# Liam-Eagen/BulletproofsPP

Measured on AMD Instinct MI355X. Metric: msm_scalar_point_pairs_per_sec, higher is better.
Workload: dtype u256 modular integer (Fq: 10x26-bit lazy limbs, Fr: 8x32-bit limbs); 1 GPU; pedersen_msm_2^20_secp256k1; pairs_per_gpu=1048576, window_bits=auto, algorithm=signed-digit Pippenger, affine in / XYZZ buckets

## Files before the change

### bulletproofspp_amd/capi.py

```python
from __future__ import annotations

import ctypes as C
import os
from typing import Optional, Sequence, Tuple

import numpy as np

_HERE = os.path.dirname(os.path.abspath(__file__))
NUM_STAGES = 6
STAGE_NAMES = ["digits", "sort", "acc_points", "acc_records", "reduce", "finish"]

SYMBOLS = [
    "bppp_ctx_create", "bppp_ctx_destroy", "bppp_ctx_set_stream", "bppp_last_error", "bppp_version",
    "bppp_msm", "bppp_msm_device", "bppp_msm_batch_device", "bppp_sum_points", "bppp_rational_reduce",
    "bppp_fold_points", "bppp_fold_points_device", "bppp_rational_reduce_eis", "bppp_fold_points_eis_device",
    "bppp_norm_round_sums_device", "bppp_lin_round_sums_device",
    "bppp_norm_round_openings_device", "bppp_lin_round_openings_device",
    "bppp_fold_scalars_device", "bppp_tensor_device", "bppp_batch_inverse_device",
    "bppp_nl_create", "bppp_nl_destroy", "bppp_nl_lengths", "bppp_nl_round_commit", "bppp_nl_round_collapse",
    "bppp_nl_get_witness", "bppp_nl_download", "bppp_nl_verify", "bppp_nl_verify_batch_device", "bppp_nl_prove", "bppp_nl_verify_challenges",
    "bppp_nlb_create", "bppp_nlb_destroy", "bppp_nlb_lengths", "bppp_nlb_round_commit", "bppp_nlb_round_collapse", "bppp_nlb_get_witness",
    "bppp_ip_create", "bppp_ip_destroy", "bppp_ip_lengths", "bppp_ip_round_commit", "bppp_ip_round_collapse", "bppp_ip_get_witness", "bppp_ip_verify", "bppp_ip_verify_batch_device",
    "bppp_lift_x_device", "bppp_device_alloc", "bppp_device_free", "bppp_upload", "bppp_download", "bppp_host_alloc", "bppp_host_free",
    "bppp_profile_enable", "bppp_profile_read",
# ... 229 lines not shown
    lib.bppp_rp_set_append.argtypes = [vp, sz, vp]
    lib.bppp_rp_set_info.argtypes = [vp, C.POINTER(C.c_uint64), C.POINTER(sz), C.POINTER(sz), C.POINTER(sz)]
    lib.bppp_rp_set_root.argtypes = [vp, vp]
    lib.bppp_rp_set_peaks.argtypes = [vp, vp]
    lib.bppp_rp_set_path_bytes.argtypes = [C.c_uint64]
    lib.bppp_rp_set_path_bytes.restype = sz
    lib.bppp_rp_set_paths.argtypes = [vp, sz, vp, vp]
    lib.bppp_rp_set_verify_paths.argtypes = [vp, sz, C.c_uint64, vp, sz, vp, vp, vp, vp, C.POINTER(C.c_int)]
    lib.bppp_seed_candidate_x.argtypes =[C.c_char_p, sz, C.c_uint64, vp]
    lib.bppp_points_from_seed.argtypes = [vp, C.c_char_p, sz, C.c_uint64, sz, vp, C.POINTER(C.c_uint64)]
    lib.bppp_points_from_seed_device.argtypes = [vp, C.c_char_p, sz, C.c_uint64, sz, vp, C.POINTER(C.c_uint64)]
    lib.bppp_rp_create_seeded.argtypes = [vp, i, i, vp, sz, vp, sz, C.c_char_p, sz, C.c_char_p, C.POINTER(vp)]
    lib.bppp_rp_create_binary_seeded.argtypes = [vp, i, i, vp, sz, vp, C.c_char_p, sz, C.c_char_p, C.POINTER(vp)]
    lib.bppp_profile_enable.argtypes = [vp, i]
    lib.bppp_profile_read.argtypes = [vp, C.POINTER(C.c_double), C.POINTER(C.c_uint64), i]
    return lib


def load_test_library() -> C.CDLL:
    p = os.path.join(_HERE, "lib", "libbppp_hip_test.so")
    if not os.path.exists(p):
        raise BpppError(f"{p} is missing: run `python -c 'import __graft_entry__ as g; g.build()'`")
    lib = C.CDLL(p)
    vp, sz, i = C.c_void_p, C.c_size_t, C.c_int
    lib.bppp_test_fe_op.argtypes = [vp, i, i, vp, vp, sz, vp]
    lib.bppp_test_point_op.argtypes = [vp, i, vp, vp, sz, vp]
    lib.bppp_test_point_quad.argtypes = [vp, i, vp, vp, sz, vp, vp]
    lib.bppp_test_fq_pair.argtypes = [vp, i, vp, vp, vp, vp, sz, vp]
    lib.bppp_test_point_chain.argtypes = [vp, i, vp, vp, sz, vp, vp]
    lib.bppp_test_mulmod_rate.argtypes = [vp, i, C.POINTER(C.c_double)]
    lib.bppp_test_last_mixed_msm_terms.argtypes = [vp, C.POINTER(C.c_uint64)]
    lib.bppp_test_last_sort_ranges.argtypes = [vp, C.POINTER(C.c_int)]
    lib.bppp_test_last_scatter_one_read.argtypes = [vp, C.POINTER(C.c_int)]
    lib.bppp_test_last_acc_sized.argtypes = [vp, C.POINTER(C.c_int)]
    lib.bppp_test_last_acc_fq29.argtypes = [vp, C.POINTER(C.c_int)]
    lib.bppp_test_fq29_op.argtypes = [vp, i, vp, vp, sz, vp, vp]
    lib.bppp_test_madd29_chain.argtypes = [vp, vp, vp, sz, sz, vp, vp]
    lib.bppp_test_madd26_chain.argtypes = [vp, vp, vp, sz, sz, vp, vp]
    lib.bppp_test_ec29_fast_op.argtypes = [vp, i, vp, sz, vp]
    lib.bppp_test_last_msm_layout.argtypes = [vp, C.POINTER(TestMsmLayout)]
    lib.bppp_test_last_msm_copy.argtypes = [vp, i, vp, sz]
    lib.bppp_test_last_windows.argtypes = [vp, C.POINTER(C.c_int)]
    lib.bppp_test_rp_last_verify_counts.argtypes = [vp, C.POINTER(C.c_uint64), C.POINTER(C.c_uint64)]
    lib.bppp_test_rp_last_block_counts.argtypes = [vp] + [C.POINTER(C.c_uint64)] * 4
    lib.bppp_test_rp_set_each_chunk.argtypes = [vp, sz]
    lib.bppp_test_rp_set_tally_short_max.argtypes = [vp, sz]
    lib.bppp_test_rp_set_tally_piece.argtypes = [vp, sz]
    lib.bppp_test_rp_set_tally_chunk.argtypes = [vp, sz]
    lib.bppp_test_rp_set_flat_chunk.argtypes = [vp, sz]
    lib.bppp_test_rp_excess_mul.argtypes = [vp, sz, vp, vp, vp]
    lib.bppp_test_rp_excess_mul2.argtypes = [vp, sz, vp, vp, vp, vp, vp]
    lib.bppp_test_rp_scan_mul.argtypes = [vp, sz, vp, vp, vp]
    lib.bppp_test_rp_scan_recode.argtypes = [vp, vp]
    lib.bppp_test_rp_scan_keys_mul.argtypes = [vp, sz, vp, sz, vp, vp]
    lib.bppp_test_rp_scan_keys_recode.argtypes = [vp, vp]
    lib.bppp_test_rp_scan_keys_geometry.argtypes = [vp, sz, sz, vp]
    lib.bppp_test_rp_witness_device.argtypes = [vp, sz, vp, vp, vp, vp, vp, vp, vp, vp, vp]
    lib.bppp_test_points_from_seed_chunked.argtypes = [vp, C.c_char_p, sz, C.c_uint64, sz, sz, vp, C.POINTER(C.c_uint64)]
    lib.bppp_test_seed_lift_digests.argtypes = [vp, C.c_char_p, sz, vp, vp, vp]
    lib.bppp_test_rp_decode_device.argtypes = [vp, sz, C.c_char_p, C.c_char_p, vp, vp, vp, vp, vp, vp]
    lib.bppp_test_comb_create.argtypes = [vp, vp, sz, i, C.POINTER(vp)]
    lib.bppp_test_comb_destroy.argtypes = [vp]
    lib.bppp_test_comb_destroy.restype = None
    lib.bppp_test_comb_msm.argtypes = [vp, vp, sz, sz, i, sz, vp]
    lib.bppp_test_comb_groups.argtypes = [vp, vp, sz, sz, sz, i, sz, vp]
    lib.bppp_test_comb_lanes.argtypes = [vp, vp, sz, sz, vp]
# ... 461 lines not shown
```

### bulletproofspp_amd/csrc/capi.hip

```cpp
#include <stdlib.h>
#include <string.h>
#include "ctx.hpp"
#include "hostmath.hpp"
#include "hosteis.hpp"

namespace bppp {
int msm_run(bppp_ctx *, const void *, const void *, size_t, size_t, int, int, uint64_t *);
int fold_points_run(bppp_ctx *, const uint64_t *, int, const uint64_t *, int, const void *, size_t, void *);
int norm_round_sums_run(bppp_ctx *, const void *, size_t, const uint64_t *, uint64_t *, uint64_t *);
int lin_round_sums_run(bppp_ctx *, const void *, const void *, size_t, uint64_t *, uint64_t *);
int round_openings_run(bppp_ctx *, const void *, size_t, int, const uint64_t *, const uint64_t *, void *, void *);
int fold_scalars_run(bppp_ctx *, const uint64_t *, const uint64_t *, const void *, size_t, void *);
int tensor_run(bppp_ctx *, const uint64_t *, size_t, const uint64_t *, const uint64_t *, size_t, void *);
int lift_x_run(bppp_ctx *, const void *, size_t, void *);
int batch_inverse_run(bppp_ctx *, const void *, size_t, int, void *);
int fold_points_eis_run(bppp_ctx *, const uint64_t *, const int *, const uint64_t *, const int *, const void *, size_t, void *);

void ctx_retain(bppp_ctx *ctx) { ctx->refs.fetch_add(1); }
void ctx_release(bppp_ctx *ctx) {
  if (ctx->refs.fetch_sub(1) != 1) return;
  hipSetDevice(ctx->device);
  hipStreamSynchronize(ctx->stream);
  if (ctx->aux_stream) hipStreamSynchronize(ctx->aux_stream);
  if (ctx->ws) hipFree(ctx->ws);
  if (ctx->ws2) hipFree(ctx->ws2);
  if (ctx->mix) hipFree(ctx->mix);
  if (ctx->pinned) hipHostFree(ctx->pinned);
  if (ctx->ev_ready) for (int i = 0; i <= BPPP_NUM_STAGES; i++) hipEventDestroy(ctx->ev[i]);
  if (ctx->aux_fork) hipEventDestroy(ctx->aux_fork);
  if (ctx->aux_join) hipEventDestroy(ctx->aux_join);
  if (ctx->aux_stream) hipStreamDestroy(ctx->aux_stream);
  if (ctx->own_stream) hipStreamDestroy(ctx->own_stream);
  delete ctx;
}
}
static int env_int(const char *name, int unset) { const char *e = getenv(name); return e ? atoi(e) : unset; }
static int env_switch(const char *name, int unset) { const char *e = getenv(name); return e ? atoi(e) != 0 : unset; }
static bool env_flag(const char *name) { return getenv(name) != nullptr; }
void MsmTune::from_env() {
  if (const char *e = getenv("BPPP_GCOST")) gcost = atof(e);
  cmin = env_int("BPPP_CMIN", 0);
  lw = env_int("BPPP_LW", 0);
  rg = env_int("BPPP_RG", 0);
  marg_s = env_int("BPPP_MARG_S", 0);
  lacc = env_int("BPPP_LACC", 0);
  window_batched = env_int("BPPP_WINDOW_BATCHED", 0);
  comb_wpe = env_int("BPPP_COMB_WPE", 0);
  comb_rows_waves = env_int("BPPP_COMB_ROWS_WAVES", 0);
  if (const char *e = getenv("BPPP_COMB_ROWS_MIN_MB")) comb_rows_min_bytes = (size_t)strtoull(e, nullptr, 10) << 20;
  small_c = env_int("BPPP_MSM_SMALL_C", 0);
  small_len = env_int("BPPP_MSM_SMALL_LEN", 0);
  small_max = env_int("BPPP_MSM_SMALL_MAX", 0);
  hist_ch = env_int("BPPP_HIST_CH", 0);
  no_small = env_flag("BPPP_MSM_NO_SMALL");
  no_balance = env_flag("BPPP_MSM_NO_BALANCE");
  sort_ranges = env_int("BPPP_SORT_RANGES", sort_ranges);
  scatter_one_read = env_switch("BPPP_SCATTER_ONE_READ", scatter_one_read);
  acc_sized = env_switch("BPPP_ACC_SIZED", acc_sized);
  acc_fq29 = env_switch("BPPP_ACC_FQ29", acc_fq29);
  acc_fast = env_switch("BPPP_ACC_FAST", acc_fast);
}
namespace bppp {
int ctx_aux(bppp_ctx *ctx) {
  if (ctx->aux_stream) return BPPP_OK;
  BPPP_HIP(ctx, hipStreamCreateWithFlags(&ctx->aux_stream, hipStreamNonBlocking));
  BPPP_HIP(ctx, hipEventCreateWithFlags(&ctx->aux_fork, hipEventDisableTiming));
  BPPP_HIP(ctx, hipEventCreateWithFlags(&ctx->aux_join, hipEventDisableTiming));
  return BPPP_OK;
}
int ensure_workspace(bppp_ctx *ctx, size_t bytes) {
  if (bytes <= ctx->ws_bytes) return BPPP_OK;
  BPPP_HIP(ctx, hipStreamSynchronize(ctx->stream));
  if (ctx->ws) BPPP_HIP(ctx, hipFree(ctx->ws));
  ctx->ws = nullptr; ctx->ws_bytes = 0;
  size_t want = bytes + bytes / 8 + (1 << 20);
  BPPP_HIP(ctx, hipMalloc(&ctx->ws, want));
  ctx->ws_bytes = want;
  return BPPP_OK;
}
int ensure_scratch(bppp_ctx *ctx, size_t bytes) {
  if (bytes <= ctx->ws2_bytes) return BPPP_OK;
  BPPP_HIP(ctx, hipStreamSynchronize(ctx->stream));
  if (ctx->ws2) BPPP_HIP(ctx, hipFree(ctx->ws2));
  ctx->ws2 = nullptr; ctx->ws2_bytes = 0;
  size_t want = bytes + bytes / 8 + (1 << 20);
  BPPP_HIP(ctx, hipMalloc(&ctx->ws2, want));
  ctx->ws2_bytes = want;
  return BPPP_OK;
}
int ensure_pinned(bppp_ctx *ctx, size_t bytes) {
// ... 268 lines not shown
```

### bulletproofspp_amd/csrc/ctx.hpp

```cpp
#pragma once
#include <hip/hip_runtime.h>
#include <stdint.h>
#include <atomic>
#include <string>
#include <vector>
#include "../../include/bppp.h"
#include "msm_plan.hpp"

struct CombLast {
  int route = -1;
  int heavy_first = 0;
  uint32_t parts = 0, tparts = 0, wsplit = 0;
  uint32_t chunks = 0, clen = 0, join_lanes = 0;
};

struct ReduceLast {
  int route = -1;
  int combine = -1;
  int c = 0, W = 0, M = 0;
  int RG = 0, Lw = 0, WPW = 0;
  int a = 0, LO = 0, HI = 0, PR = 0, PC = 0, SR = 0, SC = 0, TR = 0, TC = 0;
  int S = 0;
};

struct bppp_ctx {
  MsmTune tune;
  std::atomic<int> refs{1};
  std::atomic<bool> closed{false};
  int device = 0;
  hipStream_t stream = nullptr;
  hipStream_t own_stream = nullptr;
  hipStream_t aux_stream = nullptr;
  hipEvent_t aux_fork = nullptr, aux_join = nullptr;
  std::string err;
  void *ws = nullptr;
  size_t ws_bytes = 0;
  void *ws2 = nullptr;
  size_t ws2_bytes = 0;
  int (*pre_acc)(void *) = nullptr;
  void *pre_acc_arg = nullptr;
  void *pinned = nullptr;
  size_t pinned_bytes = 0;
  bool profile = false;
  double stage_ms[BPPP_NUM_STAGES] = {0, 0, 0, 0, 0, 0};
  uint64_t calls = 0;
  hipEvent_t ev[BPPP_NUM_STAGES + 1] = {};
  bool ev_ready = false;
  void *mix = nullptr;
  size_t mix_bytes = 0;
  uint64_t last_mixed_terms = 0;
  int last_sort_ranges = -1;
  int last_scatter_one_read = -1;
  int last_acc_sized = -1;
  int last_acc_fq29 = -1;
  int last_windows = -1;
  CombLast last_comb;
  ReduceLast last_reduce;
  bool last_msm_valid = false;
  bppp::MsmPlan last_msm_plan{};
  size_t last_msm_n = 0, last_msm_batch = 0, last_msm_table_stride = 0;
  int last_msm_shared_points = 0;
  size_t sort_lds_set = 0;
};

namespace bppp {

inline int fail(bppp_ctx *ctx, int code, const std::string &msg) {
  if (ctx) ctx->err = msg;
  return code;
}
#define BPPP_HIP(ctx, call)                                                                    \
  do {                                                                                         \
    hipError_t _e = (call);                                                                    \
    if (_e != hipSuccess)                                                                      \
      return bppp::fail(ctx, BPPP_ERR_HIP, std::string(#call) + ": " + hipGetErrorString(_e)); \
  } while (0)

void ctx_retain(bppp_ctx *ctx);
void ctx_release(bppp_ctx *ctx);
inline bool ctx_closed(const bppp_ctx *ctx) { return !ctx || ctx->closed.load(); }
int ctx_aux(bppp_ctx *ctx);
inline void ctx_drain(bppp_ctx *ctx) {
  if (ctx_closed(ctx)) return;
  hipStreamSynchronize(ctx->stream);
  if (ctx->aux_stream) hipStreamSynchronize(ctx->aux_stream);
// ... 10 lines not shown
```

### bulletproofspp_amd/csrc/msm.hip

```cpp
#include <algorithm>
#include <vector>
#include "ctx.hpp"
#include "ec.hip.h"
#include "ec29.hip.h"
#include "ec_quad.hip.h"
#include "hostcurve.hpp"
#include "hostmath.hpp"
#include "recode.hip.h"

namespace bppp {

static_assert(MSM_XYZZ_WORDS == XYZZ_WORDS, "msm_plan.hpp sizes the workspace by the stored point of ec.hip.h");
static_assert(sizeof(MsmPair) == sizeof(uint2) && sizeof(MsmQuad) == sizeof(uint4) && alignof(MsmQuad) == alignof(uint4), "the workspace's pairs and quadruples are the kernels' uint2 / uint4");

__global__ void __launch_bounds__(256) k_digits(const uint32_t *__restrict__ scalars, uint64_t total, uint32_t n, uint32_t stride, int c,
                                                int W, int acnt, int top, RecodeK K, uint16_t *__restrict__ dig,
                                                unsigned long long *__restrict__ negmask, uint32_t *__restrict__ zero, uint32_t nzero,
                                                uint32_t *__restrict__ zero2, uint32_t nzero2) {
  uint64_t i = (uint64_t)blockIdx.x * blockDim.x + threadIdx.x;
  for (uint64_t j = i; j < nzero; j += (uint64_t)gridDim.x * blockDim.x) zero[j] = 0u;
  for (uint64_t j = i; j < nzero2; j += (uint64_t)gridDim.x * blockDim.x) zero2[j] = 0u;
  bool valid = i < total;
  bool neg = false;
  if (valid) {
    uint32_t sp[9];
    neg = recode_fold(fe_load(scalars + 8 * i), K, sp);
    uint32_t inst = (uint32_t)(i / n), j = (uint32_t)(i % n);
    size_t base = (size_t)inst * W * stride + j;
    for (int w = 0; w < W; w++) {
      const int cw = w < acnt ? c : c - 1;
      const uint32_t bias = w < acnt ? 0u : (1u << (c - 2));
      const uint32_t f = recode_next(sp, cw);
      dig[base + (size_t)w * stride] = (uint16_t)(w == top ? (1u << (c - 1)) - f : f + bias);
    }
  }
  unsigned long long m = __ballot(valid && neg);
  if ((threadIdx.x & 63) == 0 && (i - (i & 63)) < total) negmask[i >> 6] = m;
}

__global__ void k_hist(const uint16_t *__restrict__ dig, uint32_t n, uint32_t stride, int c, int CH, uint32_t *__restrict__ blockhist) {
  extern __shared__ uint32_t lh[];
  const int M = 1 << (c - 1);
  const uint32_t nbw = blockIdx.x, ch = blockIdx.y;
  for (int t = threadIdx.x; t < M; t += blockDim.x) lh[t] = 0;
  __syncthreads();
  uint32_t per = (((n + CH - 1) / CH) + 7u) & ~7u, lo = ch * per, hi = min(n, lo + per);
  const uint16_t *d = dig + (size_t)nbw * stride;
  const uint32_t step = blockDim.x * 8;
  uint32_t j0 = lo + threadIdx.x * 8;
  uint4 pk = make_uint4(0u, 0u, 0u, 0u);
  if (j0 < hi) pk = *reinterpret_cast<const uint4 *>(d + j0);
  while (j0 < hi) {
    const uint32_t jn = j0 + step;
    uint4 pkn = pk;
    if (jn < hi) pkn = *reinterpret_cast<const uint4 *>(d + jn);
    uint32_t w[4] = {pk.x, pk.y, pk.z, pk.w};
#pragma unroll
    for (int k = 0; k < 8; k++) {
      int v = (int)((w[k >> 1] >> ((k & 1) * 16)) & 0xFFFFu) - M;
      if (j0 + k < hi && v) atomicAdd(&lh[(v < 0 ? -v : v) - 1], 1u);
    }
    pk = pkn; j0 = jn;
  }
  __syncthreads();
  uint32_t *out = blockhist + ((size_t)nbw * CH + ch) * M;
  for (int t = threadIdx.x; t < M; t += blockDim.x) out[t] = lh[t];
}

__global__ void __launch_bounds__(256) k_count_tiles(uint32_t *__restrict__ blockhist, int M, int CH, uint64_t FB, uint32_t *__restrict__ count,
                                                     uint32_t *__restrict__ tile_sums) {
  __shared__ uint32_t ws[4];
  const uint64_t fb = (uint64_t)blockIdx.x * 256 + threadIdx.x;
  uint32_t s = 0;
  if (fb < FB) {
    const uint64_t nbw = fb / M, mb = fb % M;
    for (int ch = 0; ch < CH; ch++) {
      const size_t at = ((size_t)nbw * CH + ch) * M + mb;
      const uint32_t t = blockhist[at];
      blockhist[at] = s;
      s += t;
    }
    count[fb] = s;
  }
  for (int d = 32; d >= 1; d >>= 1) s += __shfl_down(s, d, 64);
  if ((threadIdx.x & 63) == 0) ws[threadIdx.x >> 6] = s;
  __syncthreads();
  if (threadIdx.x == 0) atomicAdd(tile_sums + blockIdx.x / (SCAN_TILE / 256), ws[0] + ws[1] + ws[2] + ws[3]);
}
__global__ void __launch_bounds__(256) k_scan_apply(const uint32_t *__restrict__ in, uint64_t n, const uint32_t *__restrict__ tile_sums,
                                                    uint32_t *__restrict__ out, uint32_t *__restrict__ size_hist) {
  __shared__ uint32_t wsum[4], wpre[4];
  __shared__ uint32_t lh[ACC_CAP];
  if (size_hist && threadIdx.x < ACC_CAP) lh[threadIdx.x] = 0;
  uint32_t pre = 0;
  for (uint32_t i = threadIdx.x; i < blockIdx.x; i += 256) pre += tile_sums[i];
  for (int d = 32; d >= 1; d >>= 1) pre += __shfl_down(pre, d, 64);
  if ((threadIdx.x & 63) == 0) wpre[threadIdx.x >> 6] = pre;
  uint64_t base = (uint64_t)blockIdx.x * SCAN_TILE + (uint64_t)threadIdx.x * 16;
  uint32_t v[16], s = 0;
#pragma unroll
  for (int k = 0; k < 16; k++) { v[k] = (base + k < n) ? in[base + k] : 0; s += v[k]; }
  uint32_t inc = s;
  for (int d = 1; d < 64; d <<= 1) { uint32_t t = __shfl_up(inc, d, 64); if ((int)(threadIdx.x & 63) >= d) inc += t; }
  if ((threadIdx.x & 63) == 63) wsum[threadIdx.x >> 6] = inc;
  __syncthreads();
  if (size_hist) {
#pragma unroll
    for (int k = 0; k < 16; k++) {
      if (v[k] >= ACC_CAP) atomicAdd(&lh[ACC_CAP - 1], v[k] / ACC_CAP);
      if (v[k] % ACC_CAP) atomicAdd(&lh[v[k] % ACC_CAP - 1], 1u);
    }
    __syncthreads();
    if (threadIdx.x < ACC_CAP && lh[threadIdx.x]) atomicAdd(size_hist + threadIdx.x * ACC_LINE, lh[threadIdx.x]);
  }
  uint32_t woff = 0;
  for (int w = 0; w < (int)(threadIdx.x >> 6); w++) woff += wsum[w];
  uint32_t run = wpre[0] + wpre[1] + wpre[2] + wpre[3] + woff + inc - s;
#pragma unroll
  for (int k = 0; k < 16; k++) { if (base + k < n) out[base + k] = run; run += v[k]; }
  if (blockIdx.x == gridDim.x - 1 && threadIdx.x == 255) out[n] = run;
}
// ... 52 lines not shown
    }
    pk = pkn; m0 = m0n; m1 = m1n; j0 = jn;
  }
}

typedef uint32_t u32x4 __attribute__((ext_vector_type(4)));
BPPP_DI void scatter_prefetch(const uint16_t *__restrict__ d, const uint8_t *__restrict__ sgn, uint32_t j0, uint32_t step, uint32_t hi,
                              u32x4 (&pk)[SCATTER_AHEAD], uint32_t (&sneg8)[SCATTER_AHEAD]) {
#pragma unroll
  for (int i = 0; i < SCATTER_AHEAD; i++) {
    const uint32_t j = j0 + (uint32_t)i * step, ja = j < hi ? j : 0u;
    pk[i] = __builtin_nontemporal_load(reinterpret_cast<const u32x4 *>(d + ja)); sneg8[i] = sgn[ja >> 3];
  }
}
BPPP_DI void scatter_load_cursors(const uint32_t *__restrict__ bh_row, const uint32_t *__restrict__ st_row, uint32_t r0, uint32_t count, uint32_t *lh) {
  const uint4 *bh = reinterpret_cast<const uint4 *>(bh_row + r0);
  const uint4 *st = reinterpret_cast<const uint4 *>(st_row + r0);
  const uint32_t nq = count >> 2;
  for (uint32_t t0 = threadIdx.x; t0 < nq; t0 += 4 * blockDim.x) {
    uint4 a[4], b[4];
#pragma unroll
    for (int i = 0; i < 4; i++) {
      const uint32_t t = t0 + i * blockDim.x;
      a[i] = b[i] = make_uint4(0u, 0u, 0u, 0u);
      if (t < nq) { a[i] = st[t]; b[i] = bh[t]; }
    }
#pragma unroll
    for (int i = 0; i < 4; i++) {
      const uint32_t t = t0 + i * blockDim.x;
      if (t < nq) { lh[4 * t] = a[i].x + b[i].x; lh[4 * t + 1] = a[i].y + b[i].y; lh[4 * t + 2] = a[i].z + b[i].z; lh[4 * t + 3] = a[i].w + b[i].w; }
    }
  }
}
BPPP_DI void scatter_place(const u32x4 pkv, uint32_t sn, uint32_t j, uint32_t hi, uint32_t M, uint32_t r0, uint32_t Mq, uint32_t flip, uint32_t *lh, uint32_t b0,
                           uint32_t *__restrict__ sorted) {
  const uint32_t w[4] = {pkv.x, pkv.y, pkv.z, pkv.w};
#pragma unroll
  for (int e = 0; e < 8; e++) {
    int v = (int)((w[e >> 1] >> ((e & 1) * 16)) & 0xFFFFu) - (int)M;
    uint32_t mb = (uint32_t)(v < 0 ? -v : v) - 1u;
    if (j + e < hi && v && mb - r0 < Mq) {
      uint32_t sg = (v < 0 ? 1u : 0u) ^ ((sn >> e) & 1u) ^ flip;
      uint32_t pos = atomicAdd(&lh[mb - b0], 1u);
      sorted[pos] = (sg << 31) | (j + e);
    }
  }
}
__global__ void __launch_bounds__(1024) k_scatter_ranges(const uint16_t *__restrict__ dig, const unsigned long long *__restrict__ negmask, uint32_t n,
                                                         uint32_t stride, int c, int CH, int Q, uint32_t U, int top,
                                                         const uint32_t *__restrict__ blockhist, const uint32_t *__restrict__ start,
                                                         uint32_t *__restrict__ sorted) {
  extern __shared__ uint32_t lh[];
  const uint32_t M = 1u << (c - 1), Mq = M / (uint32_t)Q;
  const uint32_t s = blockIdx.x & 7u, k = blockIdx.x >> 3, u = (k / (uint32_t)CH) * 8u + s, ch = k % (uint32_t)CH;
  if (u >= U) return;
  const uint32_t nbw = u / (uint32_t)Q, r0 = (u % (uint32_t)Q) * Mq;
  const uint32_t flip = (int)nbw == top ? 1u : 0u;
  uint32_t per = (((n + CH - 1) / CH) + 7u) & ~7u, lo = ch * per, hi = min(n, lo + per);
  const uint16_t *d = dig + (size_t)nbw * stride;
  const uint8_t *sgn = reinterpret_cast<const uint8_t *>(negmask);
  const uint32_t step = blockDim.x * 8;
  uint32_t j0 = lo + threadIdx.x * 8;
  u32x4 pk[SCATTER_AHEAD];
  uint32_t sneg8[SCATTER_AHEAD];
  scatter_prefetch(d, sgn, j0, step, hi, pk, sneg8);
  scatter_load_cursors(blockhist + ((size_t)nbw * CH + ch) * M, start + (size_t)nbw * M, r0, Mq, lh);
  __syncthreads();
  for (; j0 < hi; j0 += SCATTER_AHEAD * step) {
#pragma unroll
    for (int i = 0; i < SCATTER_AHEAD; i++) {
      const uint32_t j = j0 + (uint32_t)i * step;
      if (j < hi) {
        const u32x4 pkv = pk[i];
        const uint32_t sn = sneg8[i];
        const uint32_t jn = j + SCATTER_AHEAD * step, ja = jn < hi ? jn : 0u;
        pk[i] = __builtin_nontemporal_load(reinterpret_cast<const u32x4 *>(d + ja)); sneg8[i] = sgn[ja >> 3];
        scatter_place(pkv, sn, j, hi, M, r0, Mq, flip, lh, r0, sorted);
      }
    }
  }
}

__global__ void __launch_bounds__(1024) k_scatter_one_read(const uint16_t *__restrict__ dig, const unsigned long long *__restrict__ negmask, uint32_t n,
                                                           uint32_t stride, int c, int CH, int Q, uint32_t W, int top,
                                                           const uint32_t *__restrict__ blockhist, const uint32_t *__restrict__ start,
                                                           uint32_t *__restrict__ sorted) {
  extern __shared__ uint32_t lh[];
  const uint32_t M = 1u << (c - 1);
  const uint32_t s = blockIdx.x & 7u, k = blockIdx.x >> 3, nbw = (k / (uint32_t)CH) * 8u + s, ch = k % (uint32_t)CH;
  if (nbw >= W) return;
  const uint32_t flip = (int)nbw == top ? 1u : 0u;
  uint32_t per = (((n + CH - 1) / CH) + 7u) & ~7u, lo = ch * per, hi = min(n, lo + per);
  const uint16_t *d = dig + (size_t)nbw * stride;
  const uint8_t *sgn = reinterpret_cast<const uint8_t *>(negmask);
  const uint32_t step = blockDim.x * 8, j0 = lo + threadIdx.x * 8;
  u32x4 pk[SCATTER_AHEAD];
  uint32_t sneg8[SCATTER_AHEAD];
  scatter_prefetch(d, sgn, j0, step, hi, pk, sneg8);
  scatter_load_cursors(blockhist + ((size_t)nbw * CH + ch) * M, start + (size_t)nbw * M, 0u, M, lh);
  __syncthreads();
  const uint32_t Mq = M / (uint32_t)Q;
  for (uint32_t r0 = 0; r0 < M; r0 += Mq) {
#pragma unroll
    for (int i = 0; i < SCATTER_AHEAD; i++) {
      const uint32_t j = j0 + (uint32_t)i * step;
      if (j < hi) scatter_place(pk[i], sneg8[i], j, hi, M, r0, Mq, flip, lh, 0u, sorted);
    }
    __syncthreads();
  }
}

__global__ void __launch_bounds__(256) k_acc_points(const uint32_t *__restrict__ sorted, const uint32_t *__restrict__ start, uint32_t FB,
                                                    const uint32_t *__restrict__ points, uint32_t n, uint32_t WM, int shared_pts,
                                                    int L, uint64_t G, uint32_t *__restrict__ buckets, uint32_t *__restrict__ rec_pt) {
  uint64_t g = (uint64_t)blockIdx.x * blockDim.x + threadIdx.x;
  if (g >= G) return;
  const uint32_t total = start[FB];
  const uint64_t pos0 = g * (uint64_t)L;
  if (pos0 >= total) return;
  const uint32_t pos1 = (uint32_t)min((uint64_t)total, pos0 + L);
  uint32_t lo = 0, hi = FB - 1;
  while (lo < hi) {
    const uint32_t mid = lo + (hi - lo + 1) / 2;
    if (start[mid] <= (uint32_t)pos0) lo = mid; else hi = mid - 1;
  }
  uint32_t cur = lo, end = start[cur + 1];
  const bool from_prev = start[cur] < (uint32_t)pos0;
  bool first = true;
  uint32_t e = sorted[pos0];
  xyzz acc = xyzz_inf();
  for (uint32_t p = (uint32_t)pos0; p < pos1; p++) {
    const uint32_t e_next = (p + 1 < pos1) ? sorted[p + 1] : 0u;
// ... 593 lines not shown
  for (int i = 3; i <= 5; i++) prof_mark(ctx, i);
  BPPP_HIP(ctx, hipMemcpyAsync(ctx->pinned, ws.winsum, bytes, hipMemcpyDeviceToHost, st));
  prof_mark(ctx, 6);
  BPPP_HIP(ctx, hipStreamSynchronize(st));
  window_combine_host((const uint32_t *)ctx->pinned, s.W, s.c, s.acnt, false, 0, out_xy);
  BPPP_HIP(ctx, hipGetLastError());
  prof_collect(ctx, 7);
  return BPPP_OK;
}

static int msm_sort_lds(bppp_ctx *ctx, const MsmPlan &p) {
  const size_t lds = sort_lds_bytes(p);
  if (lds > 64 * 1024 && lds > ctx->sort_lds_set) {
    BPPP_HIP(ctx, hipFuncSetAttribute((const void *)k_hist, hipFuncAttributeMaxDynamicSharedMemorySize, (int)lds));
    BPPP_HIP(ctx, hipFuncSetAttribute((const void *)k_scatter, hipFuncAttributeMaxDynamicSharedMemorySize, (int)lds));
    BPPP_HIP(ctx, hipFuncSetAttribute((const void *)k_scatter_ranges, hipFuncAttributeMaxDynamicSharedMemorySize, (int)lds));
    BPPP_HIP(ctx, hipFuncSetAttribute((const void *)k_scatter_one_read, hipFuncAttributeMaxDynamicSharedMemorySize, (int)lds));
    ctx->sort_lds_set = lds;
  }
  return BPPP_OK;
}

static void msm_digits(bppp_ctx *ctx, const MsmPlan &p, const MsmWorkspace &ws, const void *d_scalars) {
  const uint64_t total_sc = (uint64_t)p.batch * p.n;
  k_digits<<<dim3((unsigned)((total_sc + 255) / 256)), dim3(256), 0, ctx->stream>>>((const uint32_t *)d_scalars, total_sc, (uint32_t)p.n, ws.stride, p.c, p.W, p.acnt, p.top,
                                                                                     make_recode_k(p.c, p.W, p.acnt, p.top >= 0), ws.dig, ws.negmask, ws.heavy_count,
                                                                                     (uint32_t)ws.nzero, ws.tiles, (uint32_t)p.ntiles);
}

static void msm_sort(bppp_ctx *ctx, const MsmPlan &p, const MsmWorkspace &ws, size_t table_stride) {
  hipStream_t st = ctx->stream;
  const size_t lds = sort_lds_bytes(p);
  const uint32_t n = (uint32_t)p.n;
  k_hist<<<dim3((unsigned)p.NB, p.CH), dim3(p.hist_threads), lds, st>>>(ws.dig, n, ws.stride, p.c, p.CH, ws.blockhist);
  k_count_tiles<<<dim3((unsigned)((p.FB + 255) / 256)), dim3(256), 0, st>>>(ws.blockhist, p.M, p.flat ? p.W * p.CH : p.CH, p.FB, ws.count, ws.tiles);
  k_scan_apply<<<dim3(p.ntiles), dim3(256), 0, st>>>(ws.count, p.FB, ws.tiles, ws.start, ws.size_hist);
  ctx->last_sort_ranges = p.Q;
  ctx->last_windows = p.W;
  ctx->last_scatter_one_read = p.one_read ? 1 : 0;
  if (p.one_read) {
    k_scatter_one_read<<<dim3(ranged_grid(p)), dim3(p.hist_threads), lds, st>>>(ws.dig, ws.negmask, n, ws.stride, p.c, p.CH, p.Q, (uint32_t)p.W, p.top, ws.blockhist,
                                                                                ws.start, ws.sorted);
  } else if (p.Q) {
    k_scatter_ranges<<<dim3(ranged_grid(p)), dim3(p.hist_threads), ranges_lds_bytes(p), st>>>(ws.dig, ws.negmask, n, ws.stride, p.c, p.CH, p.Q, ranges_units(p), p.top,
                                                                                              ws.blockhist, ws.start, ws.sorted);
  } else
    k_scatter<<<dim3((unsigned)p.NB, p.CH), dim3(p.hist_threads), lds, st>>>(ws.dig, ws.negmask, n, ws.stride, p.c, p.CH, p.W, ws.blockhist, ws.start, ws.sorted,
                                                                             p.flat ? (uint32_t)table_stride : 0u, p.top);
}

static int msm_accumulate(bppp_ctx *ctx, const MsmPlan &p, const MsmWorkspace &ws, const void *d_points, int shared_points) {
  hipStream_t st = ctx->stream;
  uint2 *items = (uint2 *)ws.items, *heavy_items = (uint2 *)ws.heavy_items;
  uint4 *heavy_buckets = (uint4 *)ws.heavy_buckets;
  ctx->last_acc_sized = p.sized ? 1 : 0;
  ctx->last_acc_fq29 = p.fq29 ? 1 : 0;
  if (p.sized)
    k_order<<<dim3(p.ntiles), dim3(256), 0, st>>>(ws.count, p.FB, ws.size_hist, ws.cursors, items, ws.piece_base, ws.buckets, heavy_items, ws.heavy_slot, heavy_buckets,
                                                  ws.heavy_count);
  int rc = run_pre_acc(ctx); if (rc) return rc;
  if (p.sized) {
    (p.acc_fast ? k_acc_points_sized29_fast : p.fq29 ? k_acc_points_sized29 : k_acc_points_sized)<<<dim3((unsigned)((ws.items_max + 255) / 256)), dim3(256), 0, st>>>(
        ws.sorted, ws.start, ws.count, items, ws.heavy_count, ws.piece_base, (const uint32_t *)d_points, ws.buckets, ws.rec_pt);
    prof_mark(ctx, 3);
    k_merge_heavy<true><<<dim3(2048), dim3(64), 0, st>>>(ws.start, ws.count, 0, ws.rec_pt, ws.piece_base, ws.buckets, heavy_items, ws.heavy_slot, heavy_buckets,
                                                         ws.heavy_count, ws.chunk_sums);
  } else {
    k_acc_points<<<dim3((unsigned)((p.G + 255) / 256)), dim3(256), 0, st>>>(ws.sorted, ws.start, (uint32_t)p.FB, (const uint32_t *)d_points, (uint32_t)p.n,
                                                                            (uint32_t)(p.Wc * p.M), shared_points, p.L, p.G, ws.buckets, ws.rec_pt);
    prof_mark(ctx, 3);
    k_merge<<<dim3((unsigned)((p.FB + 255) / 256)), dim3(256), 0, st>>>(ws.start, ws.count, p.FB, p.L, ws.rec_pt, ws.buckets, heavy_items, ws.heavy_slot, heavy_buckets,
                                                                        ws.heavy_count);
    k_merge_heavy<false><<<dim3(2048), dim3(64), 0, st>>>(ws.start, ws.count, p.L, ws.rec_pt, nullptr, ws.buckets, heavy_items, ws.heavy_slot, heavy_buckets,
                                                          ws.heavy_count, ws.chunk_sums);
  }
  return BPPP_OK;
}

// ... 103 lines not shown
```

### bulletproofspp_amd/csrc/msm_plan.hpp

```cpp
#pragma once
#include <stddef.h>
#include <stdint.h>
#include <string.h>
#include <algorithm>

struct MsmTune {
  double gcost = 0;
  int cmin = 0;
  int lw = 0;
  int rg = 0;
  int marg_s = 0;
  int lacc = 0;
  int window_batched = 0;
  int comb_wpe = 0;
  int small_c = 0;
  int small_len = 0;
  int small_max = 0;
  int hist_ch = 0;
  int num_cus = 0;
  int sort_ranges = 4;
  int scatter_one_read = 1;
  int acc_sized = -1;
  int acc_fq29 = 1;
  int acc_fast = 1;
  bool no_small = false;
  bool no_balance = false;
  size_t comb_rows_min_bytes = (size_t)4 << 30;
  int comb_rows_waves = 0;
  void from_env();
};

namespace bppp {

struct Carver {
  char *base; size_t off = 0, cap;
  Carver(void *b, size_t c) : base((char *)b), cap(c) {}
  template <typename T> T *take(size_t count) {
    size_t bytes = (count * sizeof(T) + 255) & ~(size_t)255;
    T *p = (T *)(base ? base + off : nullptr);
    off += bytes;
    return p;
  }
};

static constexpr int MSM_XYZZ_WORDS = 40;
static constexpr int SCAN_TILE = 4096;
static constexpr uint32_t ACC_CAP = 128, ACC_LINE = 32;
static constexpr int SCATTER_AHEAD = 4;
static constexpr int MERGE_SERIAL_MAX = 8;
static constexpr int HEAVY_CHUNK = 256;
static constexpr uint32_t MSM_SMALL_MAX = 4096;
static constexpr size_t MSM_SMALL_DEFAULT_MAX = 8192;
struct MsmPair { uint32_t x, y; };
// ... 41 lines not shown
  MsmSmallPlan s;
  s.c = tune.small_c >= 5 && tune.small_c <= 8 ? tune.small_c : 6;
  const int M = 1 << (s.c - 1);
  const WindowLayout wl = window_layout(s.c, 256 % s.c != 0 && !tune.no_balance);
  s.W = wl.W; s.acnt = wl.acnt; s.top = wl.top;
  s.len = tune.small_len >= 64 && tune.small_len <= (int)MSM_SMALL_MAX ? (size_t)tune.small_len : (n <= 2048 ? 512 : 1024);
  if (n <= s.len + s.len / 2) s.len = n;
  s.S = (n + s.len - 1) / s.len;
  s.lds = (((size_t)(2 * M + 1) + s.len + (s.len + 1) / 2 + 3) & ~(size_t)3) * 4 + (size_t)(M + 4) * MSM_XYZZ_WORDS * 4;
  return s;
}
struct MsmSmallWorkspace { uint32_t *partials, *winsum; };
inline MsmSmallWorkspace carve_small(Carver &cv, const MsmSmallPlan &s) {
  MsmSmallWorkspace w;
  w.partials = cv.take<uint32_t>((size_t)s.W * s.S * MSM_XYZZ_WORDS);
  w.winsum = cv.take<uint32_t>((size_t)s.W * MSM_XYZZ_WORDS);
  return w;
}

struct MargGeom { int a, LO, HI, PR, PC, SR, SC; uint32_t row_tiles, col_tiles; int TR, TC; };

struct MsmPlan {
  size_t n, batch; int c, W, acnt, M, CH, hist_threads, Lw, WPW;
  int top;
  bool flat;
  int Wc;
  uint64_t NB, NS, FB, total_max;
  int L; uint64_t G;
  int RG;
  bool marg; MargGeom mg;
  int ntiles;
  int Q;
  bool one_read;
  bool sized;
  bool fq29;
  bool acc_fast;
};

inline void plan_windows(MsmPlan &p, size_t n, size_t batch, int c, bool flat, const MsmTune &tune) {
  p.n = n; p.batch = batch; p.c = c; p.W = 256 / c + 1; p.M = 1 << (c - 1);
  p.acnt = p.W; p.top = -1;
  if (!flat) {
    const WindowLayout l = window_layout(c, batch == 1 && c >= 3 && 256 % c != 0 && !tune.no_balance);
    p.W = l.W; p.acnt = l.acnt; p.top = l.top;
  }
  p.flat = flat; p.Wc = flat ? 1 : p.W;
  p.NB = (uint64_t)batch * p.W; p.NS = flat ? batch : p.NB; p.FB = p.NS * p.M; p.total_max = p.NB * n;
  p.ntiles = (int)((p.FB + SCAN_TILE - 1) / SCAN_TILE);
}

inline void plan_sort(MsmPlan &p, const MsmTune &tune) {
  const size_t n = p.n, batch = p.batch;
  p.hist_threads = p.M >= 8192 ? 1024 : 256;
  size_t per_block = (size_t)p.hist_threads * 64;
  p.CH = (int)std::max<size_t>(1, std::min<size_t>(64, (n + per_block - 1) / per_block));
  p.Q = 0;
  if (batch == 1 && !p.flat && (size_t)p.M * 4 > 80 * 1024 && tune.num_cus >= 8 && (tune.sort_ranges == 2 || tune.sort_ranges == 4)) {
    p.Q = tune.sort_ranges;
    const uint64_t cus = (uint64_t)tune.num_cus / 8, unit_bytes = (uint64_t)n * 4 / p.Q;
    const uint64_t ch = (cus * unit_bytes + (1u << 20) - 1) >> 20;
    p.CH = (int)std::min<uint64_t>(std::min<uint64_t>(cus, 64), std::max<uint64_t>((uint64_t)p.CH, ch));
  } else if ((size_t)p.M * 4 > 80 * 1024 && tune.num_cus > 0) {
    const double rounds = (double)p.NB * p.CH / tune.num_cus;
    if (rounds >= 0.75) {
      const uint64_t r = (uint64_t)(rounds + 0.5) ? (uint64_t)(rounds + 0.5) : 1;
      const uint64_t ch = r * (uint64_t)tune.num_cus / p.NB;
      if (ch >= 1 && ch <= 64 && 4 * ch >= 3 * (uint64_t)p.CH) p.CH = (int)ch;
    }
  }
  if (tune.hist_ch >= 1 && tune.hist_ch <= 64) p.CH = tune.hist_ch;
  const uint64_t chunk = ((((uint64_t)n + p.CH - 1) / p.CH) + 7u) & ~(uint64_t)7, lane_steps = (chunk + (uint64_t)p.hist_threads * 8 - 1) / ((uint64_t)p.hist_threads * 8);
  const uint64_t wgs = (uint64_t)p.W * p.CH, cus = (uint64_t)std::max(tune.num_cus, 1), last_round = wgs % cus;
  const bool full_rounds = wgs >= cus && !(last_round && 4 * last_round < cus);
  p.one_read = p.Q && tune.scatter_one_read && lane_steps <= (uint64_t)SCATTER_AHEAD && full_rounds;
}

inline void plan_reduce(MsmPlan &p, const MsmTune &tune) {
  if (p.M <= 64) { p.Lw = 1; p.WPW = 1; }
  else {
    p.Lw = 1;
    while (p.M / p.Lw > 64 * 64) p.Lw <<= 1;
    if (p.M / p.Lw >= 1024 && p.Lw < 4) p.Lw = std::min(4, p.M / 1024);
    if (p.Lw < 1) p.Lw = 1;
    if (tune.lw) { const int v = tune.lw; if (v >= 1 && (v & (v - 1)) == 0 && p.M / v >= 64 && p.M / v <= 4096) p.Lw = v; }
    p.WPW = p.M / p.Lw / 64;
    if (p.WPW < 1) p.WPW = 1;
  }
  p.RG = 0;
  if (p.M <= 256 && p.NS >= 4096) {
    const int cap = std::min(8, p.M);
    p.RG = std::max(1, std::min(cap, p.M / 16));
    while (p.RG < cap && p.NS * (uint64_t)p.RG < 131072) p.RG <<= 1;
    if (tune.rg) { const int v = tune.rg; if (v >= 1 && v <= cap && (v & (v - 1)) == 0) p.RG = v; }
  }
  p.marg = !p.RG && p.M >= 256 && p.NS <= 65535;
  memset(&p.mg, 0, sizeof p.mg);
  if (p.marg) {
    MargGeom &g = p.mg;
    g.a = (p.c - 1 + 1) / 2; g.LO = 1 << g.a; g.HI = p.M / g.LO;
    int S = 1;
    while (S < 16 && (2.0 * (double)p.FB) / S > 98304.0) S <<= 1;
    if (tune.marg_s) { const int v = tune.marg_s; if (v >= 1 && v <= 64 && (v & (v - 1)) == 0) S = v; }
    g.SR = std::min(S, g.LO); g.SC = std::min(S, g.HI);
    g.PR = g.LO / g.SR; g.PC = g.HI / g.SC;
    while (g.PR > 64) { g.PR >>= 1; g.SR <<= 1; }
    while (g.PC > 64) { g.PC >>= 1; g.SC <<= 1; }
    g.row_tiles = (uint32_t)(((size_t)g.HI * g.PR + 63) / 64); g.col_tiles = (uint32_t)(((size_t)g.LO * g.PC + 63) / 64);
// ... 86 lines not shown
```

### bulletproofspp_amd/csrc/testhooks.hip

```cpp
#include "../../include/bppp_test.h"
#include <vector>
#include "ctx.hpp"
#include "ec.hip.h"
#include "ec29.hip.h"
#include "ec_quad.hip.h"
#include "modinv.hip.h"
#include "fr26.hip.h"
#include "rp_internal.hpp"
#include "rpwitness.hip.h"
#include "rpdecode.hip.h"
#include "rpexcess.hip.h"
#include "rpexpart.hip.h"
#include "rpseal.hip.h"
#include "rpscan_keys.hip.h"
#include "seedpoints.hip.h"
#include "comb.hip.h"
#include "rpp_transcript.hpp"
#include "rpprove_dev.hpp"
#include "trrp.hpp"

namespace bppp {
template <int MOD> BPPP_DI fe apply_op(int op, const fe &a, const fe &b) {
  switch (op) {
    case BPPP_FE_ADD: return fe_add<MOD>(a, b);
// ... 312 lines not shown
  for (auto &w : h) { z ^= z << 13; z ^= z >> 7; z ^= z << 17; w = (uint32_t)(z >> 16); }
  for (int i = 0; i < 1024; i++) h[8 * i + 7] &= 0x7FFFFFFFu;
  hipMemcpy(seed, h.data(), h.size() * 4, hipMemcpyHostToDevice);
  hipMemset(sink, 0, 256);
  const int blocks = 256 * 4 * 8 / 4 * 2;
  hipEvent_t e0, e1; hipEventCreate(&e0); hipEventCreate(&e1);
  bppp::k_mulmod_rate<<<dim3(blocks), dim3(256), 0, ctx->stream>>>(seed, 8, sink);
  hipEventRecord(e0, ctx->stream);
  bppp::k_mulmod_rate<<<dim3(blocks), dim3(256), 0, ctx->stream>>>(seed, iters, sink);
  hipEventRecord(e1, ctx->stream);
  int rc = BPPP_OK;
  if (hipEventSynchronize(e1) != hipSuccess) rc = bppp::fail(ctx, BPPP_ERR_HIP, "mulmod_rate: kernel failed");
  float ms = 0; hipEventElapsedTime(&ms, e0, e1);
  *mulmods_per_sec = ms > 0 ? (double)blocks * 256.0 * 4.0 * iters / (ms * 1e-3) : 0.0;
  hipEventDestroy(e0); hipEventDestroy(e1); hipFree(seed); hipFree(sink);
  return rc;
}

extern "C" int bppp_test_last_mixed_msm_terms(bppp_ctx *ctx, uint64_t *terms) {
  if (!ctx || !terms) return BPPP_ERR_ARG;
  *terms = ctx->last_mixed_terms;
  return BPPP_OK;
}

extern "C" int bppp_test_last_sort_ranges(bppp_ctx *ctx, int *q) {
  if (!ctx || !q) return BPPP_ERR_ARG;
  *q = ctx->last_sort_ranges;
  return BPPP_OK;
}

extern "C" int bppp_test_last_scatter_one_read(bppp_ctx *ctx, int *one_read) {
  if (!ctx || !one_read) return BPPP_ERR_ARG;
  *one_read = ctx->last_scatter_one_read;
  return BPPP_OK;
}

extern "C" int bppp_test_last_acc_sized(bppp_ctx *ctx, int *sized) {
  if (!ctx || !sized) return BPPP_ERR_ARG;
  *sized = ctx->last_acc_sized;
  return BPPP_OK;
}

extern "C" int bppp_test_last_acc_fq29(bppp_ctx *ctx, int *fq29) {
  if (!ctx || !fq29) return BPPP_ERR_ARG;
  *fq29 = ctx->last_acc_fq29;
  return BPPP_OK;
}

extern "C" int bppp_test_fq29_op(bppp_ctx *ctx, int op, const uint32_t *a, const uint32_t *b, size_t n, uint32_t *raw, uint32_t *out) {
  if (!ctx || !a || !b || !raw || !out || op < 0 || op > 3 || n >= (1u << 24)) return BPPP_ERR_ARG;
  if (n == 0) return BPPP_OK;
  hipSetDevice(ctx->device);
  uint32_t *d = nullptr;
  if (hipMalloc(&d, n * (9 + 9 + 19 + 8) * 4) != hipSuccess) return bppp::fail(ctx, BPPP_ERR_HIP, "test_fq29_op: hipMalloc");
  uint32_t *d_b = d + n * 9, *d_raw = d_b + n * 9, *d_out = d_raw + n * 19;
  hipStream_t st = ctx->stream;
  bool ok = hipMemcpyAsync(d, a, n * 36, hipMemcpyHostToDevice, st) == hipSuccess && hipMemcpyAsync(d_b, b, n * 36, hipMemcpyHostToDevice, st) == hipSuccess;
  if (ok) k_test_fq29<<<dim3((unsigned)((n + 63) / 64)), dim3(64), 0, st>>>(op, d, d_b, (uint32_t)n, d_raw, d_out);
  ok = ok && hipMemcpyAsync(raw, d_raw, n * 19 * 4, hipMemcpyDeviceToHost, st) == hipSuccess && hipMemcpyAsync(out, d_out, n * 32, hipMemcpyDeviceToHost, st) == hipSuccess;
  if (hipStreamSynchronize(st) != hipSuccess) ok = false;
  hipFree(d);
  return ok ? BPPP_OK : bppp::fail(ctx, BPPP_ERR_HIP, "test_fq29_op: kernel or copy failed");
}
extern "C" int bppp_test_ec29_fast_op(bppp_ctx *ctx, int op, const uint32_t *in, size_t n, uint32_t *raw) {
  if (!ctx || !in || !raw || op < 0 || op > 2 || n >= (1u << 24)) return BPPP_ERR_ARG;
  if (n == 0) return BPPP_OK;
// ... 603 lines not shown
```

Measured before the change: 863.9 million pairs/s.

## Store per-chunk bucket histograms as 16-bit counts with wrap-aware prefix reconstruction

The histogram kernel now packs per-chunk bucket counts into 16-bit values, halving blockhist traffic. A new count/scan kernel processes two buckets per thread and writes 16-bit exclusive prefixes that may wrap. The scatter kernels rebuild full 32-bit cursors from the global start offsets and recover wraps by rescanning earlier chunks when a bucket's total exceeds 65535. This is enabled by default whenever ranged sorting is active and the chunk length fits in 16 bits. The cost is extra unpacking work and, for heavily loaded buckets, a serial wrap-counting loop.

```diff
diff --git a/bulletproofspp_amd/capi.py b/bulletproofspp_amd/capi.py
--- a/bulletproofspp_amd/capi.py
+++ b/bulletproofspp_amd/capi.py
@@ -285,6 +285,7 @@
     lib.bppp_test_last_mixed_msm_terms.argtypes = [vp, C.POINTER(C.c_uint64)]
     lib.bppp_test_last_sort_ranges.argtypes = [vp, C.POINTER(C.c_int)]
     lib.bppp_test_last_scatter_one_read.argtypes = [vp, C.POINTER(C.c_int)]
+    lib.bppp_test_last_hist16.argtypes = [vp, C.POINTER(C.c_int)]
     lib.bppp_test_last_acc_sized.argtypes = [vp, C.POINTER(C.c_int)]
     lib.bppp_test_last_acc_fq29.argtypes = [vp, C.POINTER(C.c_int)]
     lib.bppp_test_fq29_op.argtypes = [vp, i, vp, vp, sz, vp, vp]
diff --git a/bulletproofspp_amd/csrc/capi.hip b/bulletproofspp_amd/csrc/capi.hip
--- a/bulletproofspp_amd/csrc/capi.hip
+++ b/bulletproofspp_amd/csrc/capi.hip
@@ -56,6 +56,7 @@
   no_balance = env_flag("BPPP_MSM_NO_BALANCE");
   sort_ranges = env_int("BPPP_SORT_RANGES", sort_ranges);
   scatter_one_read = env_switch("BPPP_SCATTER_ONE_READ", scatter_one_read);
+  hist16 = env_switch("BPPP_HIST16", hist16);
   acc_sized = env_switch("BPPP_ACC_SIZED", acc_sized);
   acc_fq29 = env_switch("BPPP_ACC_FQ29", acc_fq29);
   acc_fast = env_switch("BPPP_ACC_FAST", acc_fast);
diff --git a/bulletproofspp_amd/csrc/ctx.hpp b/bulletproofspp_amd/csrc/ctx.hpp
--- a/bulletproofspp_amd/csrc/ctx.hpp
+++ b/bulletproofspp_amd/csrc/ctx.hpp
@@ -51,6 +51,7 @@
   uint64_t last_mixed_terms = 0;
   int last_sort_ranges = -1;
   int last_scatter_one_read = -1;
+  int last_hist16 = -1;
   int last_acc_sized = -1;
   int last_acc_fq29 = -1;
   int last_windows = -1;
diff --git a/bulletproofspp_amd/csrc/msm.hip b/bulletproofspp_amd/csrc/msm.hip
--- a/bulletproofspp_amd/csrc/msm.hip
+++ b/bulletproofspp_amd/csrc/msm.hip
@@ -38,7 +38,7 @@
   if ((threadIdx.x & 63) == 0 && (i - (i & 63)) < total) negmask[i >> 6] = m;
 }
 
-__global__ void k_hist(const uint16_t *__restrict__ dig, uint32_t n, uint32_t stride, int c, int CH, uint32_t *__restrict__ blockhist) {
+__global__ void k_hist(const uint16_t *__restrict__ dig, uint32_t n, uint32_t stride, int c, int CH, uint32_t *__restrict__ blockhist, int h16) {
   extern __shared__ uint32_t lh[];
   const int M = 1 << (c - 1);
   const uint32_t nbw = blockIdx.x, ch = blockIdx.y;
@@ -63,6 +63,15 @@
     pk = pkn; j0 = jn;
   }
   __syncthreads();
+  if (h16) {
+    uint4 *out16 = reinterpret_cast<uint4 *>(reinterpret_cast<uint16_t *>(blockhist) + ((size_t)nbw * CH + ch) * M);
+    const uint4 *l4 = reinterpret_cast<const uint4 *>(lh);
+    for (int t = threadIdx.x; t < M / 8; t += blockDim.x) {
+      const uint4 a = l4[2 * t], b = l4[2 * t + 1];
+      out16[t] = make_uint4(a.x | (a.y << 16), a.z | (a.w << 16), b.x | (b.y << 16), b.z | (b.w << 16));
+    }
+    return;
+  }
   uint32_t *out = blockhist + ((size_t)nbw * CH + ch) * M;
   for (int t = threadIdx.x; t < M; t += blockDim.x) out[t] = lh[t];
 }
@@ -87,6 +96,34 @@
   __syncthreads();
   if (threadIdx.x == 0) atomicAdd(tile_sums + blockIdx.x / (SCAN_TILE / 256), ws[0] + ws[1] + ws[2] + ws[3]);
 }
+__global__ void __launch_bounds__(256) k_count_tiles16(uint32_t *__restrict__ blockhist, int M, int CH, uint64_t FB, uint32_t *__restrict__ count,
+                                                       uint32_t *__restrict__ tile_sums) {
+  __shared__ uint32_t ws[4];
+  const uint64_t fb = ((uint64_t)blockIdx.x * 256 + threadIdx.x) * 2;
+  uint32_t s0 = 0, s1 = 0;
+  if (fb < FB) {
+    const uint64_t nbw = fb / M, mb = fb % M;
+    uint32_t *p = blockhist + ((size_t)nbw * CH * M + mb) / 2;
+    const size_t row = (size_t)M / 2;
+    for (int ch0 = 0; ch0 < CH; ch0 += 8) {
+      uint32_t t[8];
+#pragma unroll
+      for (int k = 0; k < 8; k++) t[k] = ch0 + k < CH ? p[(size_t)(ch0 + k) * row] : 0u;
+#pragma unroll
+      for (int k = 0; k < 8; k++)
+        if (ch0 + k < CH) {
+          p[(size_t)(ch0 + k) * row] = (s0 & 0xFFFFu) | (s1 << 16);
+          s0 += t[k] & 0xFFFFu; s1 += t[k] >> 16;
+        }
+    }
+    *reinterpret_cast<uint2 *>(count + fb) = make_uint2(s0, s1);
+  }
+  uint32_t s = s0 + s1;
+  for (int d = 32; d >= 1; d >>= 1) s += __shfl_down(s, d, 64);
+  if ((threadIdx.x & 63) == 0) ws[threadIdx.x >> 6] = s;
+  __syncthreads();
+  if (threadIdx.x == 0) atomicAdd(tile_sums + blockIdx.x / (SCAN_TILE / 512), ws[0] + ws[1] + ws[2] + ws[3]);
+}
 __global__ void __launch_bounds__(256) k_scan_apply(const uint32_t *__restrict__ in, uint64_t n, const uint32_t *__restrict__ tile_sums,
                                                     uint32_t *__restrict__ out, uint32_t *__restrict__ size_hist) {
   __shared__ uint32_t wsum[4], wpre[4];
@@ -205,6 +242,42 @@
     }
   }
 }
+BPPP_DI uint32_t scatter_wraps(const uint16_t *__restrict__ at, uint32_t ch, uint32_t M) {
+  const uint16_t *p = at - (size_t)ch * M;
+  uint32_t wraps = 0, prev = 0;
+  for (uint32_t k = 1; k <= ch; k++) { const uint32_t v = p[(size_t)k * M]; wraps += v < prev ? 1u : 0u; prev = v; }
+  return wraps;
+}
+BPPP_DI void scatter_load_cursors16(const uint16_t *__restrict__ bh_row, uint32_t ch, uint32_t M, const uint32_t *__restrict__ st_row, uint32_t r0, uint32_t count,
+                                    uint32_t *lh) {
+  const uint4 *bh = reinterpret_cast<const uint4 *>(bh_row + r0);
+  const uint4 *st = reinterpret_cast<const uint4 *>(st_row + r0);
+  uint4 *lh4 = reinterpret_cast<uint4 *>(lh);
+  const uint32_t no = count >> 3;
+  for (uint32_t t0 = threadIdx.x; t0 < no; t0 += 4 * blockDim.x) {
+    uint4 a0[4], a1[4], b[4];
+    uint32_t a2[4];
+#pragma unroll
+    for (int i = 0; i < 4; i++) {
+      const uint32_t t = t0 + i * blockDim.x;
+      a0[i] = a1[i] = b[i] = make_uint4(0u, 0u, 0u, 0u); a2[i] = 0u;
+      if (t < no) { a0[i] = st[2 * t]; a1[i] = st[2 * t + 1]; a2[i] = st_row[r0 + 8 * t + 8]; b[i] = bh[t]; }
+    }
+#pragma unroll
+    for (int i = 0; i < 4; i++) {
+      const uint32_t t = t0 + i * blockDim.x;
+      if (t < no) {
+        const uint32_t s[9] = {a0[i].x, a0[i].y, a0[i].z, a0[i].w, a1[i].x, a1[i].y, a1[i].z, a1[i].w, a2[i]};
+        uint32_t pre[8] = {b[i].x & 0xFFFFu, b[i].x >> 16, b[i].y & 0xFFFFu, b[i].y >> 16, b[i].z & 0xFFFFu, b[i].z >> 16, b[i].w & 0xFFFFu, b[i].w >> 16};
+#pragma unroll
+        for (int k = 0; k < 8; k++)
+          if (s[k + 1] - s[k] >= 65536u) pre[k] += scatter_wraps(bh_row + r0 + 8 * t + k, ch, M) << 16;
+        lh4[2 * t] = make_uint4(s[0] + pre[0], s[1] + pre[1], s[2] + pre[2], s[3] + pre[3]);
+        lh4[2 * t + 1] = make_uint4(s[4] + pre[4], s[5] + pre[5], s[6] + pre[6], s[7] + pre[7]);
+      }
+    }
+  }
+}
 BPPP_DI void scatter_place(const u32x4 pkv, uint32_t sn, uint32_t j, uint32_t hi, uint32_t M, uint32_t r0, uint32_t Mq, uint32_t flip, uint32_t *lh, uint32_t b0,
                            uint32_t *__restrict__ sorted) {
   const uint32_t w[4] = {pkv.x, pkv.y, pkv.z, pkv.w};
@@ -222,7 +295,7 @@
 __global__ void __launch_bounds__(1024) k_scatter_ranges(const uint16_t *__restrict__ dig, const unsigned long long *__restrict__ negmask, uint32_t n,
                                                          uint32_t stride, int c, int CH, int Q, uint32_t U, int top,
                                                          const uint32_t *__restrict__ blockhist, const uint32_t *__restrict__ start,
-                                                         uint32_t *__restrict__ sorted) {
+                                                         uint32_t *__restrict__ sorted, int h16) {
   extern __shared__ uint32_t lh[];
   const uint32_t M = 1u << (c - 1), Mq = M / (uint32_t)Q;
   const uint32_t s = blockIdx.x & 7u, k = blockIdx.x >> 3, u = (k / (uint32_t)CH) * 8u + s, ch = k % (uint32_t)CH;
@@ -237,7 +310,8 @@
   u32x4 pk[SCATTER_AHEAD];
   uint32_t sneg8[SCATTER_AHEAD];
   scatter_prefetch(d, sgn, j0, step, hi, pk, sneg8);
-  scatter_load_cursors(blockhist + ((size_t)nbw * CH + ch) * M, start + (size_t)nbw * M, r0, Mq, lh);
+  if (h16) scatter_load_cursors16(reinterpret_cast<const uint16_t *>(blockhist) + ((size_t)nbw * CH + ch) * M, ch, M, start + (size_t)nbw * M, r0, Mq, lh);
+  else scatter_load_cursors(blockhist + ((size_t)nbw * CH + ch) * M, start + (size_t)nbw * M, r0, Mq, lh);
   __syncthreads();
   for (; j0 < hi; j0 += SCATTER_AHEAD * step) {
 #pragma unroll
@@ -257,7 +331,7 @@
 __global__ void __launch_bounds__(1024) k_scatter_one_read(const uint16_t *__restrict__ dig, const unsigned long long *__restrict__ negmask, uint32_t n,
                                                            uint32_t stride, int c, int CH, int Q, uint32_t W, int top,
                                                            const uint32_t *__restrict__ blockhist, const uint32_t *__restrict__ start,
-                                                           uint32_t *__restrict__ sorted) {
+                                                           uint32_t *__restrict__ sorted, int h16) {
   extern __shared__ uint32_t lh[];
   const uint32_t M = 1u << (c - 1);
   const uint32_t s = blockIdx.x & 7u, k = blockIdx.x >> 3, nbw = (k / (uint32_t)CH) * 8u + s, ch = k % (uint32_t)CH;
@@ -270,7 +344,8 @@
   u32x4 pk[SCATTER_AHEAD];
   uint32_t sneg8[SCATTER_AHEAD];
   scatter_prefetch(d, sgn, j0, step, hi, pk, sneg8);
-  scatter_load_cursors(blockhist + ((size_t)nbw * CH + ch) * M, start + (size_t)nbw * M, 0u, M, lh);
+  if (h16) scatter_load_cursors16(reinterpret_cast<const uint16_t *>(blockhist) + ((size_t)nbw * CH + ch) * M, ch, M, start + (size_t)nbw * M, 0u, M, lh);
+  else scatter_load_cursors(blockhist + ((size_t)nbw * CH + ch) * M, start + (size_t)nbw * M, 0u, M, lh);
   __syncthreads();
   const uint32_t Mq = M / (uint32_t)Q;
   for (uint32_t r0 = 0; r0 < M; r0 += Mq) {
@@ -930,18 +1005,21 @@
   hipStream_t st = ctx->stream;
   const size_t lds = sort_lds_bytes(p);
   const uint32_t n = (uint32_t)p.n;
-  k_hist<<<dim3((unsigned)p.NB, p.CH), dim3(p.hist_threads), lds, st>>>(ws.dig, n, ws.stride, p.c, p.CH, ws.blockhist);
-  k_count_tiles<<<dim3((unsigned)((p.FB + 255) / 256)), dim3(256), 0, st>>>(ws.blockhist, p.M, p.flat ? p.W * p.CH : p.CH, p.FB, ws.count, ws.tiles);
+  const int h16 = p.hist16 ? 1 : 0;
+  k_hist<<<dim3((unsigned)p.NB, p.CH), dim3(p.hist_threads), lds, st>>>(ws.dig, n, ws.stride, p.c, p.CH, ws.blockhist, h16);
+  if (h16) k_count_tiles16<<<dim3((unsigned)((p.FB / 2 + 255) / 256)), dim3(256), 0, st>>>(ws.blockhist, p.M, p.CH, p.FB, ws.count, ws.tiles);
+  else k_count_tiles<<<dim3((unsigned)((p.FB + 255) / 256)), dim3(256), 0, st>>>(ws.blockhist, p.M, p.flat ? p.W * p.CH : p.CH, p.FB, ws.count, ws.tiles);
   k_scan_apply<<<dim3(p.ntiles), dim3(256), 0, st>>>(ws.count, p.FB, ws.tiles, ws.start, ws.size_hist);
   ctx->last_sort_ranges = p.Q;
   ctx->last_windows = p.W;
   ctx->last_scatter_one_read = p.one_read ? 1 : 0;
+  ctx->last_hist16 = h16;
   if (p.one_read) {
     k_scatter_one_read<<<dim3(ranged_grid(p)), dim3(p.hist_threads), lds, st>>>(ws.dig, ws.negmask, n, ws.stride, p.c, p.CH, p.Q, (uint32_t)p.W, p.top, ws.blockhist,
-                                                                                ws.start, ws.sorted);
+                                                                                ws.start, ws.sorted, h16);
   } else if (p.Q) {
     k_scatter_ranges<<<dim3(ranged_grid(p)), dim3(p.hist_threads), ranges_lds_bytes(p), st>>>(ws.dig, ws.negmask, n, ws.stride, p.c, p.CH, p.Q, ranges_units(p), p.top,
-                                                                                              ws.blockhist, ws.start, ws.sorted);
+                                                                                              ws.blockhist, ws.start, ws.sorted, h16);
   } else
     k_scatter<<<dim3((unsigned)p.NB, p.CH), dim3(p.hist_threads), lds, st>>>(ws.dig, ws.negmask, n, ws.stride, p.c, p.CH, p.W, ws.blockhist, ws.start, ws.sorted,
                                                                              p.flat ? (uint32_t)table_stride : 0u, p.top);
diff --git a/bulletproofspp_amd/csrc/msm_plan.hpp b/bulletproofspp_amd/csrc/msm_plan.hpp
--- a/bulletproofspp_amd/csrc/msm_plan.hpp
+++ b/bulletproofspp_amd/csrc/msm_plan.hpp
@@ -19,6 +19,7 @@
   int hist_ch = 0;
   int num_cus = 0;
   int sort_ranges = 4;
+  int hist16 = 1;
   int scatter_one_read = 1;
   int acc_sized = -1;
   int acc_fq29 = 1;
@@ -126,6 +127,7 @@
   int ntiles;
   int Q;
   bool one_read;
+  bool hist16;
   bool sized;
   bool fq29;
   bool acc_fast;
@@ -167,6 +169,7 @@
   const uint64_t wgs = (uint64_t)p.W * p.CH, cus = (uint64_t)std::max(tune.num_cus, 1), last_round = wgs % cus;
   const bool full_rounds = wgs >= cus && !(last_round && 4 * last_round < cus);
   p.one_read = p.Q && tune.scatter_one_read && lane_steps <= (uint64_t)SCATTER_AHEAD && full_rounds;
+  p.hist16 = p.Q && chunk <= 65535 && tune.hist16 != 0;
 }
 
 inline void plan_reduce(MsmPlan &p, const MsmTune &tune) {
diff --git a/bulletproofspp_amd/csrc/testhooks.hip b/bulletproofspp_amd/csrc/testhooks.hip
--- a/bulletproofspp_amd/csrc/testhooks.hip
+++ b/bulletproofspp_amd/csrc/testhooks.hip
@@ -368,6 +368,12 @@
 extern "C" int bppp_test_last_scatter_one_read(bppp_ctx *ctx, int *one_read) {
   if (!ctx || !one_read) return BPPP_ERR_ARG;
   *one_read = ctx->last_scatter_one_read;
+  return BPPP_OK;
+}
+
+extern "C" int bppp_test_last_hist16(bppp_ctx *ctx, int *hist16) {
+  if (!ctx || !hist16) return BPPP_ERR_ARG;
+  *hist16 = ctx->last_hist16;
   return BPPP_OK;
 }
 
```

New measurement: 882.2 million pairs/s (median of 6 runs). 2.1% higher.
